# GothiProCoder/OCR-System

Measured on AMD Instinct MI355X. Metric: pages/sec end-to-end det+rec, A4@200DPI, higher is better.
Workload: dtype bf16; 1 GPU; end-to-end det+rec, batch=64 A4@200DPI pages per GPU (BASELINE configs[3]); pages_per_gpu=64, global_batch=64, lines_last_step=3279, pages_gathered_last_step=64, parallelism=pages sharded dp1, 1 all-gather/step, ranks=1, input=pages pre-decoded (uint8 RGB) and resident in HBM when the timed region starts, det_sub_batch=64

## Files before the change

### include/lumina_ocr.h

```cpp
#ifndef LUMINA_OCR_H
#define LUMINA_OCR_H
#include <stddef.h>
#include <stdint.h>

#ifdef __cplusplus
extern "C" {
#endif

typedef struct lumina_ocr lumina_ocr_t;

#define LUMINA_REC_H 32
#define LUMINA_REC_W 320
#define LUMINA_REC_T 80
#define LUMINA_MAX_WORDS 40
#define LUMINA_MAX_BOXES 1000

int lumina_ocr_create(int device, lumina_ocr_t** out);
void lumina_ocr_destroy(lumina_ocr_t* h);
const char* lumina_ocr_last_error(const lumina_ocr_t* h);
const char* lumina_ocr_version(void);
int lumina_ocr_set_option(lumina_ocr_t* h, const char* key, int value);

int lumina_ocr_load_det_weights(lumina_ocr_t* h, const void* blob, size_t nbytes);
int lumina_ocr_load_rec_weights(lumina_ocr_t* h, const void* blob, size_t nbytes);
// ... 27 lines not shown
int lumina_ocr_rec_forward(lumina_ocr_t* h, const uint8_t* crops_dev, const int32_t* widths_dev, int n_crops, int32_t* idx_dev,
                           float* prob_dev, void* stream);

int lumina_ocr_ctc_decode(lumina_ocr_t* h, const int32_t* idx_dev, const float* prob_dev, int n, int32_t* text_dev, int32_t* len_dev,
                          float* score_dev, void* stream);

int lumina_ocr_ctc_decode_words(lumina_ocr_t* h, const int32_t* idx_dev, const float* prob_dev, int n, const int32_t* quads_dev,
                                const int32_t* widths_dev, const int32_t* flip_dev , int space_id, int32_t* text_dev,
                                int32_t* len_dev, float* score_dev, int32_t* word_quads_dev, int32_t* word_span_dev, float* word_score_dev,
                                int32_t* word_count_dev, void* stream);

int lumina_ocr_resize_lanczos(lumina_ocr_t* h, const uint8_t* in_dev, int n, int height, int width, int channels, uint8_t* out_dev,
                              int out_h, int out_w, void* stream);
int lumina_ocr_enhance(lumina_ocr_t* h, const uint8_t* img_dev, int n, int height, int width, float contrast, float sharpness,
                       uint8_t* tmp_dev, uint8_t* out_dev, void* stream);

int lumina_ocr_binarize(lumina_ocr_t* h, const uint8_t* img_dev, int n, int height, int width, int adaptive, int threshold, uint8_t* out_dev,
                        void* stream);

int lumina_ocr_exif_transpose(lumina_ocr_t* h, const uint8_t* img_dev, int n, int height, int width, int orientation, uint8_t* out_dev, void* stream);
int lumina_ocr_grayscale(lumina_ocr_t* h, const uint8_t* img_dev, int n, int height, int width, uint8_t* out_dev, void* stream);
int lumina_ocr_denoise(lumina_ocr_t* h, const uint8_t* img_dev, int n, int height, int width, uint8_t* out_dev, void* stream);

int lumina_ocr_deskew(lumina_ocr_t* h, const uint8_t* pages_dev, int n, int height, int width, uint8_t* out_dev, double* rot_dev,
                      int32_t* info_dev, uint8_t* edges_dev, int32_t* segs_dev, int32_t* nsegs_dev, void* stream);
int lumina_ocr_deskew_warp(lumina_ocr_t* h, const uint8_t* pages_dev, int n, int height, int width, const double* rot_dev, uint8_t* out_dev,
                           void* stream);

int lumina_ocr_table_rules(lumina_ocr_t* h, const uint8_t* pages_dev, int n, int height, int width, int threshold, int gap, int min_len,
                           int max_thick, int max_rules, int32_t* hrules_dev, int32_t* vrules_dev, int32_t* counts_dev, uint64_t* hmask_dev,
// ... 50 lines not shown
```

### ocr-system_amd/csrc/capi.hip

```cpp
#include <cstdlib>
#include <cstring>
#include <new>

#include "../../include/lumina_ocr.h"
#include "dbpost.h"
#include "deskew.h"
#include "engine.h"
#include "marks.h"
#include "ops.h"
#include "orient.h"
#include "resize.h"
#include "runs.h"
#include "jpeg.h"
#include "jpegdec.h"
#include "pngdec.h"
#include "stem_conv.h"
#include "tables.h"

#define API_TRY try {
#define API_CATCH(h)                                                             \
    }                                                                            \
    catch (const std::exception& e) { return locr_fail(h, "exception", e.what()); } \
    catch (...) { return locr_fail(h, "exception", "unknown"); }

// ... 84 lines not shown
    else if (!strcmp(key, "fuse_head")) h->fuse_head = value != 0;
    else if (!strcmp(key, "fuse_mb")) h->fuse_mb = value != 0;
    else if (!strcmp(key, "fuse_pool")) h->fuse_pool = value != 0;
    else if (!strcmp(key, "fuse_stem")) h->fuse_stem = value != 0;
    else if (!strcmp(key, "fpn_multi")) h->fpn_multi = value != 0;
    else if (!strcmp(key, "fpn_compose")) h->fpn_compose = value != 0;
    else if (!strcmp(key, "fuse_short")) h->fuse_short = value != 0;
    else if (!strcmp(key, "conv_ring")) h->conv_ring = value != 0;
    else if (!strcmp(key, "blocked_layout")) h->blocked_layout = value != 0;
    else if (!strcmp(key, "conv_big_min")) h->conv_big_min = value >= 0 ? value : 1024;
    else if (!strcmp(key, "ring_orient")) h->ring_orient = value < 0 ? -1 : (value != 0);
    else if (!strcmp(key, "post_group")) h->post_group = value > 0 ? value : 1;
    else if (!strcmp(key, "tail_group")) h->tail_group = value > 0 ? value : 0;
    else if (!strcmp(key, "svtr_f16")) h->svtr_f16 = value < 0 ? -1 : (value != 0);
    else if (!strcmp(key, "png_sub_batch_mb")) h->pd_sub_batch_mb = value > 0 ? value : 1;
    else if (!strcmp(key, "conv2d_variant")) h->conv2d_variant = value < 0 || value > 2 ? 0 : value;
    else return locr_fail(h, "set_option: unknown key", key);
    return 0;
}

int lumina_ocr_load_det_weights(lumina_ocr_t* h, const void* blob, size_t nbytes) {
    if (!h || !blob) return 1;
    BIND(h);
    API_TRY return eng_load_det(h, blob, nbytes); API_CATCH(h)
}
int lumina_ocr_load_rec_weights(lumina_ocr_t* h, const void* blob, size_t nbytes) {
    if (!h || !blob) return 1;
    BIND(h);
    API_TRY return eng_load_rec(h, blob, nbytes); API_CATCH(h)
}
// ... 194 lines not shown
    auto it = h->coeff_cache.find(key);
    if (it == h->coeff_cache.end()) {
        std::vector<int> bounds, kk;
        lumina_ocr::Coeffs c;
        lanczos_coeffs(in_size, out_size, &c.ksize, &bounds, &kk);
        c.bounds_host = std::make_shared<std::vector<int>>(bounds);
        c.bounds = static_cast<int*>(eng_upload(h, bounds.data(), bounds.size() * 4));
        c.kk = static_cast<int*>(eng_upload(h, kk.data(), kk.size() * 4));
        if (!c.bounds || !c.kk) return locr_fail(h, "resize", "coefficient table upload");
        it = h->coeff_cache.emplace(key, c).first;
    }
    *out = it->second;
    return 0;
}

int lumina_ocr_resize_lanczos(lumina_ocr_t* h, const uint8_t* in_dev, int n, int height, int width, int channels, uint8_t* out_dev,
                              int out_h, int out_w, void* stream) {
    if (!h || !in_dev || !out_dev || n <= 0 || height <= 0 || width <= 0 || out_h <= 0 || out_w <= 0 || channels <= 0)
        return locr_fail(h, "resize_lanczos", "bad arguments");
    BIND(h);
    API_TRY
    hipStream_t st = (hipStream_t)stream;
    const uint8_t* src = in_dev;
    int cur_w = width;
    const bool need_h = out_w != width, need_v = out_h != height;
    if (!need_h && !need_v) {
        return hip_rc(h, "resize_lanczos", hipMemcpyAsync(out_dev, in_dev, (size_t)n * height * width * channels, hipMemcpyDeviceToDevice, st));
    }
    if (need_h) {
        lumina_ocr::Coeffs c;
        if (get_coeffs(h, width, out_w, &c)) return 1;
        uint8_t* dst = out_dev;
        if (need_v) {
            if (hip_rc(h, "resize_lanczos", h->aux.reserve((size_t)n * height * out_w * channels))) return 1;
            dst = h->aux.get();
        }
        if (hip_rc(h, "resize_lanczos", resample_launch(src, dst, c.bounds, c.kk, c.ksize, n, height, width, channels, out_w, 0, c.bounds_host->data(), st))) return 1;
        src = dst; cur_w = out_w;
    }
    if (need_v) {
        lumina_ocr::Coeffs c;
        if (get_coeffs(h, height, out_h, &c)) return 1;
        if (hip_rc(h, "resize_lanczos", resample_launch(src, out_dev, c.bounds, c.kk, c.ksize, n, height, cur_w, channels, out_h, 1, c.bounds_host->data(), st))) return 1;
    }
    return 0;
    API_CATCH(h)
}

int lumina_ocr_enhance(lumina_ocr_t* h, const uint8_t* img_dev, int n, int height, int width, float contrast, float sharpness,
                       uint8_t* tmp_dev, uint8_t* out_dev, void* stream) {
    if (!h || !img_dev || !tmp_dev || !out_dev || n <= 0) return locr_fail(h, "enhance", "bad arguments");
    BIND(h);
    if (hip_rc(h, "enhance", h->sums.reserve(sizeof(unsigned long long) * (size_t)n))) return 1;
    unsigned long long* sums = reinterpret_cast<unsigned long long*>(h->sums.get());
    return hip_rc(h, "enhance", enhance_launch(img_dev, tmp_dev, out_dev, sums, n, height, width, contrast, sharpness, (hipStream_t)stream));
}

int lumina_ocr_binarize(lumina_ocr_t* h, const uint8_t* img_dev, int n, int height, int width, int adaptive, int threshold, uint8_t* out_dev, void* stream) {
    if (!h || !img_dev || !out_dev || n <= 0 || height <= 0 || width <= 0) return locr_fail(h, "binarize", "bad arguments");
    BIND(h);
    return hip_rc(h, "binarize", binarize_launch(img_dev, out_dev, n, height, width, adaptive != 0, threshold, (hipStream_t)stream));
}

int lumina_ocr_exif_transpose(lumina_ocr_t* h, const uint8_t* img_dev, int n, int height, int width, int orientation, uint8_t* out_dev, void* stream) {
    if (!h || !img_dev || !out_dev || n <= 0 || height <= 0 || width <= 0 || orientation < 1 || orientation > 8 || img_dev == out_dev)
        return locr_fail(h, "exif_transpose", "bad arguments (orientation 1..8, not in place)");
    BIND(h);
    return hip_rc(h, "exif_transpose", exif_transpose_launch(img_dev, out_dev, n, height, width, orientation, (hipStream_t)stream));
}

// ... 280 lines not shown
```

### ocr-system_amd/csrc/engine.h

```cpp
#pragma once
#include <map>
#include <memory>
#include <string>
#include <type_traits>
#include <vector>

#include "common.h"
#include "conv_mfma.h"
#include "mbconv.h"
#include "svtr.h"

struct Tensor4 {
    bf16_t* p = nullptr;
    int n = 0, h = 0, w = 0, c = 0;
    bool blk = false;
    int n_src = 0; const bf16_t* xs[4] = {nullptr, nullptr, nullptr, nullptr}; int xs_shift[4] = {0, 0, 0, 0};
    int xs_c[4] = {0, 0, 0, 0}, xs_cs[4] = {0, 0, 0, 0};
    int src_c(int k) const { return xs_c[k] ? xs_c[k] : c / n_src; }
    int src_cs(int k) const { return xs_cs[k] ? xs_cs[k] : src_c(k); }
    size_t elems() const { return (size_t)n * h * w * c; }
};

struct ConvLayer {
    std::string name;
// ... 103 lines not shown
    bool blocked_layout = true;
    bool conv_ring = true;
    int svtr_f16 = -1;
    int conv2d_variant = 0;
    int ring_orient = -1;
    bool fuse_short = true;
    bool fpn_compose = true;
    bool fpn_multi = true;
    bool fuse_stem = true;
    bool fuse_mb = true;
    bool time_convs = false;
    std::vector<LaunchRecord> launches;
    struct Coeffs { int ksize = 0; int* bounds = nullptr; int* kk = nullptr; std::shared_ptr<std::vector<int>> bounds_host; };
    std::map<std::pair<int, int>, Coeffs> coeff_cache;
    Growable<DeviceMem> aux;
    Growable<DeviceMem> sums;
    int jd_last_passes = 0;
    struct Staging { Growable<PinnedMem> buf; Event uploaded; };
    Staging jd_stage[2];
    int jd_stage_next = 0;
    Staging pd_stage;
    int pd_sub_batch_mb = 768;
    float* dk_trig = nullptr; short* dk_wtab = nullptr;
};

int locr_fail(lumina_ocr* eng, const char* what, const char* detail);
bool parse_blob(lumina_ocr* eng, const void* blob, size_t n, std::map<std::string, HostBlobTensor>* out);

int eng_load_det(lumina_ocr* eng, const void* blob, size_t n);
int eng_load_rec(lumina_ocr* eng, const void* blob, size_t n);
int eng_det_forward(lumina_ocr* eng, const uint8_t* pages, int B, int H, int W, int Hp, int Wp, bf16_t* prob, hipStream_t st);
// ... 11 lines not shown
```

### ocr-system_amd/csrc/resize.h

```cpp
#pragma once
#include <vector>

#include "common.h"

void lanczos_coeffs(int in_size, int out_size, int* ksize_out, std::vector<int>* bounds, std::vector<int>* kk);
hipError_t resample_launch(const uint8_t* in, uint8_t* out, const int* bounds_dev, const int* kk_dev, int ksize, int N, int H, int W, int C,
                           int out_len, int axis, const int* bounds_host, hipStream_t st);
hipError_t enhance_launch(const uint8_t* img, uint8_t* tmp, uint8_t* out, unsigned long long* sums_dev, int N, int H, int W, float contrast,
                          float sharpness, hipStream_t st);
hipError_t binarize_launch(const uint8_t* img, uint8_t* out, int N, int H, int W, int adaptive, int threshold, hipStream_t st);
hipError_t grayscale_launch(const uint8_t* img, uint8_t* out, int N, int H, int W, hipStream_t st);
hipError_t median3_launch(const uint8_t* img, uint8_t* out, int N, int H, int W, hipStream_t st);
hipError_t exif_transpose_launch(const uint8_t* img, uint8_t* out, int N, int H, int W, int orientation, hipStream_t st);
```

### ocr-system_amd/csrc/resize.hip

```cpp
#include "resize.h"
#include "lds_rows.h"

#include <cmath>

namespace {

constexpr int PRECISION_BITS = 32 - 8 - 2;

__global__ __launch_bounds__(256) void resample_h_kernel(const uint8_t* in, uint8_t* out, const int* bounds, const int* kk, int ksize, int H, int W,
                                                         int C, int Wo, size_t total_bytes) {
    extern __shared__ uint32_t row_lds[];
    const int row = blockIdx.x;
    const size_t start = (size_t)row * W * C;
    const int off = (int)(start & 3);
    const uint32_t* src = reinterpret_cast<const uint32_t*>(in + (start - off));
    const int nwords = (off + W * C + 3) >> 2;
    const size_t wbase = start - off;
    for (int i = threadIdx.x; i < nwords; i += 256) {
        uint32_t w;
        if (wbase + 4 * (size_t)(i + 1) <= total_bytes) w = src[i];
        else {
            w = 0;
            for (int b = 0; b < 4; ++b)
                if (wbase + 4 * (size_t)i + b < total_bytes) w |= (uint32_t)in[wbase + 4 * (size_t)i + b] << (8 * b);
// ... 167 lines not shown
            const uint32_t w = __builtin_amdgcn_alignbyte(lr[1], lr[0], (uint32_t)(off & 3));
            const int kj = kl[rr * VK + j];
            s0 += __mul24((int)(w & 0xff), kj); s1 += __mul24((int)((w >> 8) & 0xff), kj); s2 += __mul24((int)((w >> 16) & 0xff), kj); s3 += __mul24((int)(w >> 24), kj);
        }
        s0 >>= PRECISION_BITS; s1 >>= PRECISION_BITS; s2 >>= PRECISION_BITS; s3 >>= PRECISION_BITS;
        const uint32_t res = (uint32_t)(s0 < 0 ? 0 : (s0 > 255 ? 255 : s0)) | ((uint32_t)(s1 < 0 ? 0 : (s1 > 255 ? 255 : s1)) << 8) |
                             ((uint32_t)(s2 < 0 ? 0 : (s2 > 255 ? 255 : s2)) << 16) | ((uint32_t)(s3 < 0 ? 0 : (s3 > 255 ? 255 : s3)) << 24);
        uint8_t* dst = out + go - mo + 4 * tid;
        if (ew >= 0 && ew + 4 <= rowbytes) *reinterpret_cast<uint32_t*>(dst) = res;
        else
            for (int j = 0; j < 4; ++j)
                if (ew + j >= 0 && ew + j < rowbytes) dst[j] = (uint8_t)(res >> (8 * j));
    }
}

__global__ __launch_bounds__(256) void gray_sum_kernel(const uint8_t* img, unsigned long long* sums, int HW) {
    __shared__ unsigned long long part[4];
    const int n = blockIdx.y;
    const uint8_t* p = img + (size_t)n * HW * 3;
    unsigned long long s = 0;
    for (int i = blockIdx.x * blockDim.x + threadIdx.x; i < HW; i += gridDim.x * blockDim.x) {
        const unsigned r = p[(size_t)i * 3], g = p[(size_t)i * 3 + 1], b = p[(size_t)i * 3 + 2];
        s += (r * 19595u + g * 38470u + b * 7471u + 0x8000u) >> 16;
    }
    for (int m = 32; m >= 1; m >>= 1) {
        const unsigned lo = __shfl_xor((unsigned)(s & 0xffffffffull), m), hi = __shfl_xor((unsigned)(s >> 32), m);
        s += ((unsigned long long)hi << 32) | lo;
    }
    if ((threadIdx.x & 63) == 0) part[threadIdx.x >> 6] = s;
    __syncthreads();
// ... 171 lines not shown
        if (bounds_host != nullptr && ksize <= VKMAX && lds_bytes <= 60 * 1024) {
            const dim3 grid((rowbytes + 3 + VT_XB - 1) / VT_XB, (out_len + VT_R - 1) / VT_R, N);
            if (vk == 9) hipLaunchKernelGGL(resample_v_tile_kernel<9>, grid, dim3(256), lds_bytes, st, in, out, bounds_dev, kk_dev, ksize, H, rowbytes, out_len, (long long)N * H * rowbytes);
            else hipLaunchKernelGGL(resample_v_tile_kernel<VKMAX>, grid, dim3(256), lds_bytes, st, in, out, bounds_dev, kk_dev, ksize, H, rowbytes, out_len, (long long)N * H * rowbytes);
            return hipGetLastError();
        }
        const bool a4 = rowbytes % 4 == 0 && (reinterpret_cast<uintptr_t>(in) % 4 == 0) && (reinterpret_cast<uintptr_t>(out) % 4 == 0);
        const bool a2 = rowbytes % 2 == 0 && (reinterpret_cast<uintptr_t>(in) % 2 == 0) && (reinterpret_cast<uintptr_t>(out) % 2 == 0);
        if (a4) hipLaunchKernelGGL(resample_v_kernel<4>, dim3(N * out_len), dim3(256), 0, st, in, out, bounds_dev, kk_dev, ksize, H, rowbytes, out_len);
        else if (a2) hipLaunchKernelGGL(resample_v_kernel<2>, dim3(N * out_len), dim3(256), 0, st, in, out, bounds_dev, kk_dev, ksize, H, rowbytes, out_len);
        else hipLaunchKernelGGL(resample_v_kernel<1>, dim3(N * out_len), dim3(256), 0, st, in, out, bounds_dev, kk_dev, ksize, H, rowbytes, out_len);
    }
    return hipGetLastError();
}

namespace {
constexpr int BZ_TH = 16, BZ_TW = 64, BZ_R = 5;
__constant__ float c_gauss11[11] = {0x1.20c256p-7f, 0x1.bcb86ap-6f, 0x1.0ab50ap-4f, 0x1.f2464cp-4f, 0x1.6a7e1ep-3f, 0x1.9ac20ap-3f,
                                    0x1.6a7e1ep-3f, 0x1.f2464cp-4f, 0x1.0ab50ap-4f, 0x1.bcb86ap-6f, 0x1.20c256p-7f};
__device__ __forceinline__ int lum_L(const uint8_t* p) { return (19595 * p[0] + 38470 * p[1] + 7471 * p[2] + 0x8000) >> 16; }

__global__ __launch_bounds__(256) void binarize_kernel(const uint8_t* img, uint8_t* out, int H, int W, int adaptive, int threshold) {
    __shared__ uint8_t sL[(BZ_TH + 2 * BZ_R) * (BZ_TW + 2 * BZ_R)];
    __shared__ float sRow[(BZ_TH + 2 * BZ_R) * BZ_TW];
    const int pg = blockIdx.z, y0 = blockIdx.y * BZ_TH, x0 = blockIdx.x * BZ_TW, tid = threadIdx.x;
    const uint8_t* src = img + (size_t)pg * H * W * 3;
    uint8_t* dst = out + (size_t)pg * H * W * 3;
    constexpr int LW = BZ_TW + 2 * BZ_R, LH = BZ_TH + 2 * BZ_R;
    if (!adaptive) {
        for (int i = tid; i < BZ_TH * BZ_TW; i += 256) {
// ... 102 lines not shown
    long long g = (npix + 255) / 256;
    hipLaunchKernelGGL(grayscale_kernel, dim3((unsigned)(g > 65536 ? 65536 : g)), dim3(256), 0, st, img, out, npix);
    return hipGetLastError();
}

hipError_t median3_launch(const uint8_t* img, uint8_t* out, int N, int H, int W, hipStream_t st) {
    hipLaunchKernelGGL(median3_kernel, dim3((W + 63) / 64, (H + 3) / 4, N), dim3(256), 0, st, img, out, H, W);
    return hipGetLastError();
}

hipError_t binarize_launch(const uint8_t* img, uint8_t* out, int N, int H, int W, int adaptive, int threshold, hipStream_t st) {
    hipLaunchKernelGGL(binarize_kernel, dim3((W + BZ_TW - 1) / BZ_TW, (H + BZ_TH - 1) / BZ_TH, N), dim3(256), 0, st, img, out, H, W, adaptive, threshold);
    return hipGetLastError();
}

hipError_t enhance_launch(const uint8_t* img, uint8_t* tmp, uint8_t* out, unsigned long long* sums_dev, int N, int H, int W, float contrast,
                          float sharpness, hipStream_t st) {
    hipError_t e = hipMemsetAsync(sums_dev, 0, sizeof(unsigned long long) * N, st);
    if (e != hipSuccess) return e;
    const int HW = H * W;
    int gx = (HW + 255) / 256;
    if (gx > 2048) gx = 2048;
    hipLaunchKernelGGL(gray_sum_kernel, dim3(gx > 64 ? 64 : gx, N), dim3(256), 0, st, img, sums_dev, HW);
    (void)tmp;
    const int rowb = W * 3;
    hipLaunchKernelGGL(enhance_kernel, dim3((rowb + 3 + EN_XB - 1) / EN_XB, (H + EN_R - 1) / EN_R, N), dim3(256), 0, st, img, out, sums_dev, H, W,
                       contrast, sharpness, (long long)N * H * rowb);
    return hipGetLastError();
}
```

### ocr-system_amd/lumina_ocr/engine.py

```python
from __future__ import annotations

import ctypes
import os
from pathlib import Path
from typing import Dict, Optional, Tuple

import numpy as np

from . import arch

_LIB_PATH = Path(__file__).resolve().parent.parent / "lib" / "liblumina_ocr.so"

REC_H, REC_W, REC_T = 32, 320, 80
MAX_WORDS = 40
MAX_BOXES = 1000


class EngineUnavailable(RuntimeError):
    pass


class EngineError(RuntimeError):
    pass

# ... 25 lines not shown
        "lumina_ocr_det_postprocess": (i32, [vp, vp, i32, i32, i32, i32, i32, f32, f32, f32, i32, i32, vp, vp, vp, vp]),
        "lumina_ocr_rec_crop": (i32, [vp, vp, i32, i32, i32, vp, vp, i32, vp, vp, vp]),
        "lumina_ocr_rec_crop_oriented": (i32, [vp, vp, i32, i32, i32, vp, vp, i32, vp, vp, vp, vp]),
        "lumina_ocr_cls_crop": (i32, [vp, vp, i32, i32, i32, vp, vp, i32, vp, vp, vp]),
        "lumina_ocr_load_cls_weights": (i32, [vp, vp, sz]),
        "lumina_ocr_cls_forward": (i32, [vp, vp, vp, i32, f32, vp, vp, vp, vp]),
        "lumina_ocr_rec_forward": (i32, [vp, vp, vp, i32, vp, vp, vp]),
        "lumina_ocr_ctc_decode": (i32, [vp, vp, vp, i32, vp, vp, vp, vp]),
        "lumina_ocr_ctc_decode_words": (i32, [vp, vp, vp, i32, vp, vp, vp, i32, vp, vp, vp, vp, vp, vp, vp, vp]),
        "lumina_ocr_conv2d": (i32, [vp, vp, i32, i32, i32, i32, vp, vp, i32, i32, i32, i32, vp, vp, vp]),
        "lumina_ocr_read_tap": (i32, [vp, c.c_char_p, vp, sz, c.POINTER(i32)]),
        "lumina_ocr_conv_timing": (i32, [vp, c.POINTER(c.c_double), c.POINTER(c.c_double), c.POINTER(i32)]),
        "lumina_ocr_conv_timing_detail": (i32, [vp, c.c_char_p, sz]),
        "lumina_ocr_resize_lanczos": (i32, [vp, vp, i32, i32, i32, i32, vp, i32, i32, vp]),
        "lumina_ocr_enhance": (i32, [vp, vp, i32, i32, i32, f32, f32, vp, vp, vp]),
        "lumina_ocr_jpeg_encode": (i32, [vp, vp, i32, i32, i32, i32, i32, vp, sz, vp, vp]),
        "lumina_ocr_jpeg_probe": (i32, [vp, sz, vp]),
        "lumina_ocr_jpeg_last_passes": (i32, [vp]),
        "lumina_ocr_jpeg_decode_async": (i32, [vp, vp, vp, i32, i32, i32, vp, vp, i32, vp]),
        "lumina_ocr_jpeg_decode": (i32, [vp, vp, vp, i32, i32, i32, vp, vp, vp]),
        "lumina_ocr_jpeg_coefficients": (i32, [vp, vp, i32, i32, i32, i32, vp, vp]),
        "lumina_ocr_png_probe": (i32, [vp, sz, vp]),
        "lumina_ocr_png_decode": (i32, [vp, vp, vp, i32, i32, i32, vp, vp, vp]),
        "lumina_ocr_load_svtr_weights": (i32, [vp, vp, sz]),
        "lumina_ocr_svtr_forward": (i32, [vp, vp, vp, i32, vp, vp, vp]),
        "lumina_ocr_svtr_num_classes": (i32, [vp]),
        "lumina_ocr_svtr_dtype": (i32, [vp]),
        "lumina_ocr_binarize": (i32, [vp, vp, i32, i32, i32, i32, i32, vp, vp]),
        "lumina_ocr_grayscale": (i32, [vp, vp, i32, i32, i32, vp, vp]),
        "lumina_ocr_exif_transpose": (i32, [vp, vp, i32, i32, i32, i32, vp, vp]),
# ... 16 lines not shown
            missing.append(name)
            continue
        fn.restype = res
        fn.argtypes = args
    lib._missing = missing
    _lib = lib
    return lib


EXPORTED_SYMBOLS = [
    "lumina_ocr_create", "lumina_ocr_destroy", "lumina_ocr_last_error", "lumina_ocr_version", "lumina_ocr_set_option",
    "lumina_ocr_load_det_weights", "lumina_ocr_load_rec_weights", "lumina_ocr_num_classes", "lumina_ocr_normalize",
    "lumina_ocr_det_forward", "lumina_ocr_det_postprocess", "lumina_ocr_rec_crop", "lumina_ocr_rec_crop_oriented", "lumina_ocr_cls_crop",
    "lumina_ocr_load_cls_weights", "lumina_ocr_cls_forward", "lumina_ocr_rec_forward",
    "lumina_ocr_ctc_decode", "lumina_ocr_ctc_decode_words", "lumina_ocr_conv2d", "lumina_ocr_read_tap", "lumina_ocr_conv_timing", "lumina_ocr_conv_timing_detail",
    "lumina_ocr_resize_lanczos", "lumina_ocr_enhance", "lumina_ocr_jpeg_encode", "lumina_ocr_jpeg_coefficients", "lumina_ocr_jpeg_probe", "lumina_ocr_jpeg_decode", "lumina_ocr_jpeg_decode_async", "lumina_ocr_jpeg_last_passes",
    "lumina_ocr_png_probe", "lumina_ocr_png_decode",
    "lumina_ocr_load_svtr_weights", "lumina_ocr_svtr_forward", "lumina_ocr_svtr_num_classes", "lumina_ocr_svtr_dtype", "lumina_ocr_binarize", "lumina_ocr_exif_transpose", "lumina_ocr_grayscale", "lumina_ocr_denoise", "lumina_ocr_deskew", "lumina_ocr_deskew_warp",
    "lumina_ocr_table_rules", "lumina_ocr_selection_marks", "lumina_ocr_rules_and_marks",
    "lumina_ocr_page_quarter_workspace_bytes", "lumina_ocr_page_quarter", "lumina_ocr_page_turn", "lumina_ocr_page_vote",
]


def _torch():
    import torch
    return torch


def _ptr(t) -> int:
    return 0 if t is None else t.data_ptr()

# ... 295 lines not shown
        buf = ctypes.create_string_buffer(1 << 20)
        self._chk(self.lib.lumina_ocr_conv_timing_detail(self._h, buf, len(buf)))
        rows = []
        for line in buf.value.decode().splitlines():
            name, kern, ms, gf, mb = line.split()
            rows.append((name, kern, float(ms), float(gf), float(mb)))
        return rows

    def resize_lanczos(self, img, out_h: int, out_w: int):
        torch = _torch()
        n, h, w, c = img.shape
        out = torch.empty((n, out_h, out_w, c), dtype=torch.uint8, device=img.device)
        self._chk(self.lib.lumina_ocr_resize_lanczos(self._h, _ptr(img), n, h, w, c, _ptr(out), out_h, out_w, self._stream()))
        return out

    def deskew(self, pages, debug: bool = False, estimate_only: bool = False):
        torch = _torch()
        n, h, w, c = pages.shape
        assert c == 3 and pages.dtype == torch.uint8 and pages.is_contiguous()
        out = None if estimate_only else torch.empty_like(pages)
        rot = torch.empty((n, 3), dtype=torch.float64, device=pages.device)
        info = torch.empty((n, 2), dtype=torch.int32, device=pages.device)
        edges = segs = nsegs = None
        if debug:
            edges = torch.empty((n, h, w), dtype=torch.uint8, device=pages.device)
            segs = torch.zeros((n, 512, 8, 4), dtype=torch.int32, device=pages.device)
            nsegs = torch.zeros((n, 512), dtype=torch.int32, device=pages.device)
        self._chk(self.lib.lumina_ocr_deskew(self._h, _ptr(pages), n, h, w, _ptr(out), _ptr(rot), _ptr(info), _ptr(edges), _ptr(segs), _ptr(nsegs),
                                             self._stream()))
        return (out, rot, info, edges, segs, nsegs) if debug else (out, rot)
# ... 141 lines not shown
```

### ocr-system_amd/lumina_ocr/pipeline.py

```python
from __future__ import annotations

import logging
from dataclasses import dataclass, field
from typing import List, Optional, Sequence, Tuple

import numpy as np

from . import arch
from .engine import MAX_BOXES, Engine
from .utils import page_orient
from .utils.image_preprocessing import get_optimal_size

logger = logging.getLogger(__name__)


@dataclass
class PageDetections:
    quads: np.ndarray
    texts: List[str]
    scores: np.ndarray
    det_scores: np.ndarray
    width: int = 0
    height: int = 0
    text_ids: Optional[np.ndarray] = None
# ... 56 lines not shown
        self.mark_params = dict(arch.MARK_PARAMS if mark_params is None else mark_params)
        self.page_orient = bool(page_orient)
        self.word_boxes = bool(word_boxes)
        self.space_id = self.charset.index(" ") if " " in self.charset else -1
        self.page_orient_params = dict(arch.PAGE_ORIENT_PARAMS if page_orient_params is None else page_orient_params)
        if self.angle_cls and not engine.cls_loaded:
            raise ValueError("angle_cls needs the orientation classifier's weights (Engine.load_cls)")
        if self.page_orient and not engine.cls_loaded:
            raise ValueError("page_orient needs the orientation classifier's weights (Engine.load_cls)")
        if self.page_orient and gather is not None:
            raise ValueError("page_orient does not run with a gather: a page's turn and its processed size stay on their rank")

    def preprocess(self, pages, enhance: bool = True, deskew: bool = False):
        b, h, w, _ = pages.shape
        nw, nh = get_optimal_size(w, h, self.max_dimension)
        x = pages if (nw, nh) == (w, h) else self.eng.resize_lanczos(pages, nh, nw)
        if deskew:
            x, self.last_skew_angles = self.eng.deskew(x)
        if self.binarize:
            return self.eng.binarize(x, adaptive=self.binarize == "adaptive")
        return self.eng.enhance(x, 1.2, 1.1) if enhance else x

    def detect(self, processed):
        b, h, w, _ = processed.shape
        prob = self.eng.det_forward(processed)
        return self.eng.det_postprocess(prob, h, w, **self.post)

    def recognize(self, processed, boxes, scores, counts) -> List[PageDetections]:
        return self.finish(self.submit_recognize(processed, boxes, scores, counts))[0]

# ... 239 lines not shown
```

Before: 1540 pages/sec.

## Fuse two-pass Lanczos resize with grayscale sum into one LDS-tiled kernel

```diff
diff --git a/include/lumina_ocr.h b/include/lumina_ocr.h
--- a/include/lumina_ocr.h
+++ b/include/lumina_ocr.h
@@ -65,6 +65,9 @@
                               int out_h, int out_w, void* stream);
 int lumina_ocr_enhance(lumina_ocr_t* h, const uint8_t* img_dev, int n, int height, int width, float contrast, float sharpness,
                        uint8_t* tmp_dev, uint8_t* out_dev, void* stream);
+int lumina_ocr_preprocess(lumina_ocr_t* h, const uint8_t* in_dev, int n, int height, int width, uint8_t* resized_dev, uint8_t* out_dev, int out_h,
+                          int out_w, float contrast, float sharpness, void* stream);
+int lumina_ocr_debug_preprocess_state(lumina_ocr_t* h, unsigned long long* sums_host, int n, int* resize_path);
 
 int lumina_ocr_binarize(lumina_ocr_t* h, const uint8_t* img_dev, int n, int height, int width, int adaptive, int threshold, uint8_t* out_dev,
                         void* stream);
diff --git a/ocr-system_amd/csrc/capi.hip b/ocr-system_amd/csrc/capi.hip
--- a/ocr-system_amd/csrc/capi.hip
+++ b/ocr-system_amd/csrc/capi.hip
@@ -122,6 +122,7 @@
     else if (!strcmp(key, "tail_group")) h->tail_group = value > 0 ? value : 0;
     else if (!strcmp(key, "svtr_f16")) h->svtr_f16 = value < 0 ? -1 : (value != 0);
     else if (!strcmp(key, "png_sub_batch_mb")) h->pd_sub_batch_mb = value > 0 ? value : 1;
+    else if (!strcmp(key, "resize_fused")) h->resize_fused = value != 0;
     else if (!strcmp(key, "conv2d_variant")) h->conv2d_variant = value < 0 || value > 2 ? 0 : value;
     else return locr_fail(h, "set_option: unknown key", key);
     return 0;
@@ -346,36 +347,54 @@
     return 0;
 }
 
+static int resize_run(lumina_ocr* h, const uint8_t* in_dev, int n, int height, int width, int channels, uint8_t* out_dev, int out_h, int out_w,
+                      unsigned long long* sums_dev, bool* sums_done, const uint8_t** result, hipStream_t st) {
+    *sums_done = false;
+    h->last_resize_path = 0;
+    const bool need_h = out_w != width, need_v = out_h != height;
+    const size_t out_bytes = (size_t)n * out_h * out_w * channels;
+    const size_t inter = need_h && need_v ? ((size_t)n * height * out_w * channels + 255) / 256 * 256 : 0;
+    lumina_ocr::Coeffs ch, cv;
+    if (need_h && get_coeffs(h, width, out_w, &ch)) return 1;
+    if (need_v && get_coeffs(h, height, out_h, &cv)) return 1;
+    ResampleHvPlan plan;
+    if (need_h && need_v && h->resize_fused) plan = resample_hv_plan(ch.ksize, ch.bounds_host->data(), cv.ksize, cv.bounds_host->data(), n, channels, out_h, out_w);
+    const size_t aux_bytes = (plan.ok ? 0 : inter) + (out_dev ? 0 : out_bytes);
+    if (aux_bytes && hip_rc(h, "resize_lanczos", h->aux.reserve(aux_bytes))) return 1;
+    if (!out_dev) out_dev = h->aux.get() + (plan.ok ? 0 : inter);
+    *result = out_dev;
+    if (!need_h && !need_v) {
+        return hip_rc(h, "resize_lanczos", hipMemcpyAsync(out_dev, in_dev, out_bytes, hipMemcpyDeviceToDevice, st));
+    }
+    if (plan.ok) {
+        if (hip_rc(h, "resize_lanczos", resample_hv_launch(plan, in_dev, out_dev, ch.bounds, ch.kk, ch.ksize, cv.bounds, cv.kk, cv.ksize, n, height, width,
+                                                           out_h, out_w, sums_dev, st))) return 1;
+        *sums_done = sums_dev != nullptr;
+        h->last_resize_path = 1;
+        return 0;
+    }
+    const uint8_t* src = in_dev;
+    int cur_w = width;
+    if (need_h) {
+        uint8_t* dst = need_v ? h->aux.get() : out_dev;
+        if (hip_rc(h, "resize_lanczos", resample_launch(src, dst, ch.bounds, ch.kk, ch.ksize, n, height, width, channels, out_w, 0, ch.bounds_host->data(), st))) return 1;
+        src = dst; cur_w = out_w;
+    }
+    if (need_v) {
+        if (hip_rc(h, "resize_lanczos", resample_launch(src, out_dev, cv.bounds, cv.kk, cv.ksize, n, height, cur_w, channels, out_h, 1, cv.bounds_host->data(), st))) return 1;
+    }
+    return 0;
+}
+
 int lumina_ocr_resize_lanczos(lumina_ocr_t* h, const uint8_t* in_dev, int n, int height, int width, int channels, uint8_t* out_dev,
                               int out_h, int out_w, void* stream) {
     if (!h || !in_dev || !out_dev || n <= 0 || height <= 0 || width <= 0 || out_h <= 0 || out_w <= 0 || channels <= 0)
         return locr_fail(h, "resize_lanczos", "bad arguments");
     BIND(h);
     API_TRY
-    hipStream_t st = (hipStream_t)stream;
-    const uint8_t* src = in_dev;
-    int cur_w = width;
-    const bool need_h = out_w != width, need_v = out_h != height;
-    if (!need_h && !need_v) {
-        return hip_rc(h, "resize_lanczos", hipMemcpyAsync(out_dev, in_dev, (size_t)n * height * width * channels, hipMemcpyDeviceToDevice, st));
-    }
-    if (need_h) {
-        lumina_ocr::Coeffs c;
-        if (get_coeffs(h, width, out_w, &c)) return 1;
-        uint8_t* dst = out_dev;
-        if (need_v) {
-            if (hip_rc(h, "resize_lanczos", h->aux.reserve((size_t)n * height * out_w * channels))) return 1;
-            dst = h->aux.get();
-        }
-        if (hip_rc(h, "resize_lanczos", resample_launch(src, dst, c.bounds, c.kk, c.ksize, n, height, width, channels, out_w, 0, c.bounds_host->data(), st))) return 1;
-        src = dst; cur_w = out_w;
-    }
-    if (need_v) {
-        lumina_ocr::Coeffs c;
-        if (get_coeffs(h, height, out_h, &c)) return 1;
-        if (hip_rc(h, "resize_lanczos", resample_launch(src, out_dev, c.bounds, c.kk, c.ksize, n, height, cur_w, channels, out_h, 1, c.bounds_host->data(), st))) return 1;
-    }
-    return 0;
+    bool sums_done;
+    const uint8_t* result;
+    return resize_run(h, in_dev, n, height, width, channels, out_dev, out_h, out_w, nullptr, &sums_done, &result, (hipStream_t)stream);
     API_CATCH(h)
 }
 
@@ -385,7 +404,36 @@
     BIND(h);
     if (hip_rc(h, "enhance", h->sums.reserve(sizeof(unsigned long long) * (size_t)n))) return 1;
     unsigned long long* sums = reinterpret_cast<unsigned long long*>(h->sums.get());
-    return hip_rc(h, "enhance", enhance_launch(img_dev, tmp_dev, out_dev, sums, n, height, width, contrast, sharpness, (hipStream_t)stream));
+    return hip_rc(h, "enhance", enhance_launch(img_dev, tmp_dev, out_dev, sums, false, n, height, width, contrast, sharpness, (hipStream_t)stream));
+}
+
+int lumina_ocr_preprocess(lumina_ocr_t* h, const uint8_t* in_dev, int n, int height, int width, uint8_t* resized_dev, uint8_t* out_dev, int out_h,
+                          int out_w, float contrast, float sharpness, void* stream) {
+    if (!h || !in_dev || !out_dev || n <= 0 || height <= 0 || width <= 0 || out_h <= 0 || out_w <= 0 || resized_dev == out_dev)
+        return locr_fail(h, "preprocess", "bad arguments");
+    BIND(h);
+    API_TRY
+    hipStream_t st = (hipStream_t)stream;
+    if (hip_rc(h, "preprocess", h->sums.reserve(sizeof(unsigned long long) * (size_t)n))) return 1;
+    unsigned long long* sums = reinterpret_cast<unsigned long long*>(h->sums.get());
+    const uint8_t* resized = in_dev;
+    bool sums_done = false;
+    if (out_h != height || out_w != width) {
+        if (hip_rc(h, "preprocess", hipMemsetAsync(sums, 0, sizeof(unsigned long long) * (size_t)n, st))) return 1;
+        if (resize_run(h, in_dev, n, height, width, 3, resized_dev, out_h, out_w, sums, &sums_done, &resized, st)) return 1;
+    }
+    return hip_rc(h, "preprocess", enhance_launch(resized, nullptr, out_dev, sums, sums_done, n, out_h, out_w, contrast, sharpness, st));
+    API_CATCH(h)
+}
+
+int lumina_ocr_debug_preprocess_state(lumina_ocr_t* h, unsigned long long* sums_host, int n, int* resize_path) {
+    if (!h || (sums_host && n <= 0)) return locr_fail(h, "debug_preprocess_state", "bad arguments");
+    BIND(h);
+    if (resize_path) *resize_path = h->last_resize_path;
+    if (!sums_host) return 0;
+    if (!h->sums.get() || h->sums.cap < sizeof(unsigned long long) * (size_t)n) return locr_fail(h, "debug_preprocess_state", "no enhance / preprocess call of that many pages yet");
+    if (hipDeviceSynchronize() != hipSuccess) return locr_fail(h, "debug_preprocess_state", "sync failed");
+    return hip_rc(h, "debug_preprocess_state", hipMemcpy(sums_host, h->sums.get(), sizeof(unsigned long long) * (size_t)n, hipMemcpyDeviceToHost));
 }
 
 int lumina_ocr_binarize(lumina_ocr_t* h, const uint8_t* img_dev, int n, int height, int width, int adaptive, int threshold, uint8_t* out_dev, void* stream) {
diff --git a/ocr-system_amd/csrc/engine.h b/ocr-system_amd/csrc/engine.h
--- a/ocr-system_amd/csrc/engine.h
+++ b/ocr-system_amd/csrc/engine.h
@@ -141,7 +141,9 @@
     struct Coeffs { int ksize = 0; int* bounds = nullptr; int* kk = nullptr; std::shared_ptr<std::vector<int>> bounds_host; };
     std::map<std::pair<int, int>, Coeffs> coeff_cache;
     Growable<DeviceMem> aux;
+    bool resize_fused = true;
     Growable<DeviceMem> sums;
+    int last_resize_path = -1;
     int jd_last_passes = 0;
     struct Staging { Growable<PinnedMem> buf; Event uploaded; };
     Staging jd_stage[2];
diff --git a/ocr-system_amd/csrc/resize.h b/ocr-system_amd/csrc/resize.h
--- a/ocr-system_amd/csrc/resize.h
+++ b/ocr-system_amd/csrc/resize.h
@@ -6,8 +6,13 @@
 void lanczos_coeffs(int in_size, int out_size, int* ksize_out, std::vector<int>* bounds, std::vector<int>* kk);
 hipError_t resample_launch(const uint8_t* in, uint8_t* out, const int* bounds_dev, const int* kk_dev, int ksize, int N, int H, int W, int C,
                            int out_len, int axis, const int* bounds_host, hipStream_t st);
-hipError_t enhance_launch(const uint8_t* img, uint8_t* tmp, uint8_t* out, unsigned long long* sums_dev, int N, int H, int W, float contrast,
-                          float sharpness, hipStream_t st);
+struct ResampleHvPlan { bool ok = false; int p_in = 0, nr_max = 0; size_t lds_bytes = 0; };
+ResampleHvPlan resample_hv_plan(int ksize_h, const int* bounds_h_host, int ksize_v, const int* bounds_v_host, int N, int C, int Ho, int Wo);
+hipError_t resample_hv_launch(const ResampleHvPlan& p, const uint8_t* in, uint8_t* out, const int* bounds_h_dev, const int* kk_h_dev, int ksize_h,
+                              const int* bounds_v_dev, const int* kk_v_dev, int ksize_v, int N, int H, int W, int Ho, int Wo,
+                              unsigned long long* sums_dev, hipStream_t st);
+hipError_t enhance_launch(const uint8_t* img, uint8_t* tmp, uint8_t* out, unsigned long long* sums_dev, bool sums_given, int N, int H, int W,
+                          float contrast, float sharpness, hipStream_t st);
 hipError_t binarize_launch(const uint8_t* img, uint8_t* out, int N, int H, int W, int adaptive, int threshold, hipStream_t st);
 hipError_t grayscale_launch(const uint8_t* img, uint8_t* out, int N, int H, int W, hipStream_t st);
 hipError_t median3_launch(const uint8_t* img, uint8_t* out, int N, int H, int W, hipStream_t st);
diff --git a/ocr-system_amd/csrc/resize.hip b/ocr-system_amd/csrc/resize.hip
--- a/ocr-system_amd/csrc/resize.hip
+++ b/ocr-system_amd/csrc/resize.hip
@@ -205,6 +205,113 @@
     }
 }
 
+constexpr int FT_X = 84, FT_Y = 40, FP_MID = 67;
+template <int FK>
+__global__ __launch_bounds__(256) void resample_hv_rgb_kernel(const uint8_t* in, uint8_t* out, const int* __restrict__ bounds_h,
+                                                              const int* __restrict__ kk_h, int ksize_h, const int* __restrict__ bounds_v,
+                                                              const int* __restrict__ kk_v, int ksize_v, int H, int W, int Ho, int Wo, int p_in,
+                                                              int nr_max, long long total_in, unsigned long long* sums) {
+    constexpr int FW = (3 * FK + 3 + 3) / 4;
+    extern __shared__ uint32_t lds[];
+    __shared__ unsigned part[4];
+    uint32_t* lin = lds;
+    uint32_t* mid = lds + nr_max * p_in;
+    const int tid = threadIdx.x;
+    const int n = blockIdx.z, yo0 = blockIdx.y * FT_Y, xo0 = blockIdx.x * FT_X;
+    const int nx = min(FT_X, Wo - xo0), ny = min(FT_Y, Ho - yo0);
+    const int rgrp = tid / FT_X, xi = tid - rgrp * FT_X;
+    const int xo = xo0 + min(xi, nx - 1);
+    const int lo = bounds_h[2 * xo];
+    int kreg[FK];
+#pragma unroll
+    for (int j = 0; j < FK; ++j) kreg[j] = j < ksize_h ? kk_h[(size_t)xo * ksize_h + j] : 0;
+    const int px_lo = bounds_h[2 * xo0];
+    const int px_hi = bounds_h[2 * (xo0 + nx - 1)] + bounds_h[2 * (xo0 + nx - 1) + 1];
+    const int r_lo = bounds_v[2 * yo0];
+    const int nr = bounds_v[2 * (yo0 + ny - 1)] + bounds_v[2 * (yo0 + ny - 1) + 1] - r_lo;
+    const int rowb = W * 3;
+    const long long g0 = (((long long)n * H + r_lo) * W + px_lo) * 3;
+    const int nw = ((px_hi - px_lo) * 3 + 3 + 3) / 4;
+    fill_rows(lin, p_in, nw, in, g0, rowb, nr, 0, nr, total_in, WordIdentity());
+    __syncthreads();
+    const uintptr_t ibase = reinterpret_cast<uintptr_t>(in), obase = reinterpret_cast<uintptr_t>(out);
+    const int m0 = (int)((ibase + (unsigned long long)g0) & 3), dm = rowb & 3;
+    if (rgrp < 3 && xi < nx) {
+        uint8_t* mb = reinterpret_cast<uint8_t*>(mid) + 4 + xi * 3;
+        const int pb = (lo - px_lo) * 3;
+#pragma unroll 2
+        for (int r = rgrp; r < nr; r += 3) {
+            const int off = ((m0 + r * dm) & 3) + pb;
+            const uint32_t* lr = lin + r * p_in + (off >> 2);
+            const uint32_t sh = (uint32_t)(off & 3);
+            uint32_t w[FW];
+#pragma unroll
+            for (int i = 0; i < FW; ++i) w[i] = lr[i];
+            uint32_t a[FW - 1];
+#pragma unroll
+            for (int i = 0; i < FW - 1; ++i) a[i] = __builtin_amdgcn_alignbyte(w[i + 1], w[i], sh);
+            int s0 = 1 << (PRECISION_BITS - 1), s1 = s0, s2 = s0;
+#pragma unroll
+            for (int j = 0; j < FK; ++j) {
+                s0 += __mul24((int)((a[(3 * j) >> 2] >> (8 * ((3 * j) & 3))) & 0xffu), kreg[j]);
+                s1 += __mul24((int)((a[(3 * j + 1) >> 2] >> (8 * ((3 * j + 1) & 3))) & 0xffu), kreg[j]);
+                s2 += __mul24((int)((a[(3 * j + 2) >> 2] >> (8 * ((3 * j + 2) & 3))) & 0xffu), kreg[j]);
+            }
+            s0 >>= PRECISION_BITS; s1 >>= PRECISION_BITS; s2 >>= PRECISION_BITS;
+            uint8_t* o = mb + r * (FP_MID * 4);
+            o[0] = (uint8_t)(s0 < 0 ? 0 : (s0 > 255 ? 255 : s0));
+            o[1] = (uint8_t)(s1 < 0 ? 0 : (s1 > 255 ? 255 : s1));
+            o[2] = (uint8_t)(s2 < 0 ? 0 : (s2 > 255 ? 255 : s2));
+        }
+    }
+    __syncthreads();
+    const int wv = __builtin_amdgcn_readfirstlane(tid >> 6), lane = tid & 63;
+    const int segb = nx * 3;
+    unsigned gs = 0;
+    for (int rr = wv; rr < ny; rr += 4) {
+        const int yo = yo0 + rr;
+        const int vlo = bounds_v[2 * yo] - r_lo;
+        const int* kv = kk_v + (size_t)yo * ksize_v;
+        const long long go = (((long long)n * Ho + yo) * Wo + xo0) * 3;
+        const int mo = (int)((obase + (unsigned long long)go) & 3);
+        const int b0 = 4 * lane - mo;
+        const int off = 4 + b0;
+        const uint32_t* lr = mid + vlo * FP_MID + (off >> 2);
+        const uint32_t sh = (uint32_t)(off & 3);
+        int s0 = 1 << (PRECISION_BITS - 1), s1 = s0, s2 = s0, s3 = s0;
+#pragma unroll
+        for (int j = 0; j < FK; ++j) {
+            const uint32_t w = __builtin_amdgcn_alignbyte(lr[j * FP_MID + 1], lr[j * FP_MID], sh);
+            const int kj = j < ksize_v ? kv[j] : 0;
+            s0 += __mul24((int)(w & 0xff), kj); s1 += __mul24((int)((w >> 8) & 0xff), kj); s2 += __mul24((int)((w >> 16) & 0xff), kj); s3 += __mul24((int)(w >> 24), kj);
+        }
+        s0 >>= PRECISION_BITS; s1 >>= PRECISION_BITS; s2 >>= PRECISION_BITS; s3 >>= PRECISION_BITS;
+        const uint32_t res = (uint32_t)(s0 < 0 ? 0 : (s0 > 255 ? 255 : s0)) | ((uint32_t)(s1 < 0 ? 0 : (s1 > 255 ? 255 : s1)) << 8) |
+                             ((uint32_t)(s2 < 0 ? 0 : (s2 > 255 ? 255 : s2)) << 16) | ((uint32_t)(s3 < 0 ? 0 : (s3 > 255 ? 255 : s3)) << 24);
+        uint8_t* dst = out + go + b0;
+        if (b0 >= 0 && b0 + 4 <= segb) *reinterpret_cast<uint32_t*>(dst) = res;
+        else
+            for (int j = 0; j < 4; ++j)
+                if (b0 + j >= 0 && b0 + j < segb) dst[j] = (uint8_t)(res >> (8 * j));
+        if (sums != nullptr) {
+            const uint32_t nxt = (uint32_t)__shfl_down((int)res, 1);
+            const int d = (3 - (b0 + 3) % 3) % 3;
+            const uint32_t p1 = __builtin_amdgcn_alignbyte(nxt, res, (uint32_t)d);
+            const uint32_t p2 = __builtin_amdgcn_alignbyte(nxt, res, 3u);
+            const unsigned l1 = ((p1 & 0xff) * 19595u + ((p1 >> 8) & 0xff) * 38470u + ((p1 >> 16) & 0xff) * 7471u + 0x8000u) >> 16;
+            const unsigned l2 = ((p2 & 0xff) * 19595u + ((p2 >> 8) & 0xff) * 38470u + ((p2 >> 16) & 0xff) * 7471u + 0x8000u) >> 16;
+            if (b0 + d >= 0 && b0 + d < segb) gs += l1;
+            if (d == 0 && b0 + 3 < segb) gs += l2;
+        }
+    }
+    if (sums != nullptr) {
+        for (int m = 32; m >= 1; m >>= 1) gs += __shfl_xor(gs, m);
+        if (lane == 0) part[wv] = gs;
+        __syncthreads();
+        if (tid == 0) atomicAdd(&sums[n], (unsigned long long)part[0] + part[1] + part[2] + part[3]);
+    }
+}
+
 __global__ __launch_bounds__(256) void gray_sum_kernel(const uint8_t* img, unsigned long long* sums, int HW) {
     __shared__ unsigned long long part[4];
     const int n = blockIdx.y;
@@ -406,6 +513,38 @@
     return hipGetLastError();
 }
 
+ResampleHvPlan resample_hv_plan(int ksize_h, const int* bounds_h_host, int ksize_v, const int* bounds_v_host, int N, int C, int Ho, int Wo) {
+    constexpr int FK = 9, FW = (3 * FK + 3 + 3) / 4;
+    ResampleHvPlan p;
+    if (C != 3 || ksize_h > FK || ksize_v > FK || bounds_h_host == nullptr || bounds_v_host == nullptr || N > 65535) return p;
+    int npx_max = 0, nr_max = 0;
+    for (int x0 = 0; x0 < Wo; x0 += FT_X) {
+        const int x1 = (x0 + FT_X < Wo ? x0 + FT_X : Wo) - 1;
+        const int sp = bounds_h_host[2 * x1] + bounds_h_host[2 * x1 + 1] - bounds_h_host[2 * x0];
+        if (sp > npx_max) npx_max = sp;
+    }
+    for (int y0 = 0; y0 < Ho; y0 += FT_Y) {
+        const int y1 = (y0 + FT_Y < Ho ? y0 + FT_Y : Ho) - 1;
+        const int sp = bounds_v_host[2 * y1] + bounds_v_host[2 * y1 + 1] - bounds_v_host[2 * y0];
+        if (sp > nr_max) nr_max = sp;
+    }
+    p.p_in = ((3 + 3 * npx_max) / 4 + FW + 1) | 1;
+    p.nr_max = nr_max;
+    p.lds_bytes = ((size_t)nr_max * p.p_in + (size_t)(nr_max + FK) * FP_MID) * 4;
+    p.ok = p.lds_bytes <= 48 * 1024;
+    return p;
+}
+
+hipError_t resample_hv_launch(const ResampleHvPlan& p, const uint8_t* in, uint8_t* out, const int* bounds_h_dev, const int* kk_h_dev, int ksize_h,
+                              const int* bounds_v_dev, const int* kk_v_dev, int ksize_v, int N, int H, int W, int Ho, int Wo,
+                              unsigned long long* sums_dev, hipStream_t st) {
+    if (!p.ok) return hipErrorInvalidValue;
+    const dim3 grid((Wo + FT_X - 1) / FT_X, (Ho + FT_Y - 1) / FT_Y, N);
+    hipLaunchKernelGGL(resample_hv_rgb_kernel<9>, grid, dim3(256), p.lds_bytes, st, in, out, bounds_h_dev, kk_h_dev, ksize_h, bounds_v_dev, kk_v_dev,
+                       ksize_v, H, W, Ho, Wo, p.p_in, p.nr_max, (long long)N * H * W * 3, sums_dev);
+    return hipGetLastError();
+}
+
 namespace {
 constexpr int BZ_TH = 16, BZ_TW = 64, BZ_R = 5;
 __constant__ float c_gauss11[11] = {0x1.20c256p-7f, 0x1.bcb86ap-6f, 0x1.0ab50ap-4f, 0x1.f2464cp-4f, 0x1.6a7e1ep-3f, 0x1.9ac20ap-3f,
@@ -538,14 +677,16 @@
     return hipGetLastError();
 }
 
-hipError_t enhance_launch(const uint8_t* img, uint8_t* tmp, uint8_t* out, unsigned long long* sums_dev, int N, int H, int W, float contrast,
-                          float sharpness, hipStream_t st) {
-    hipError_t e = hipMemsetAsync(sums_dev, 0, sizeof(unsigned long long) * N, st);
-    if (e != hipSuccess) return e;
-    const int HW = H * W;
-    int gx = (HW + 255) / 256;
-    if (gx > 2048) gx = 2048;
-    hipLaunchKernelGGL(gray_sum_kernel, dim3(gx > 64 ? 64 : gx, N), dim3(256), 0, st, img, sums_dev, HW);
+hipError_t enhance_launch(const uint8_t* img, uint8_t* tmp, uint8_t* out, unsigned long long* sums_dev, bool sums_given, int N, int H, int W,
+                          float contrast, float sharpness, hipStream_t st) {
+    if (!sums_given) {
+        hipError_t e = hipMemsetAsync(sums_dev, 0, sizeof(unsigned long long) * N, st);
+        if (e != hipSuccess) return e;
+        const int HW = H * W;
+        int gx = (HW + 255) / 256;
+        if (gx > 2048) gx = 2048;
+        hipLaunchKernelGGL(gray_sum_kernel, dim3(gx > 64 ? 64 : gx, N), dim3(256), 0, st, img, sums_dev, HW);
+    }
     (void)tmp;
     const int rowb = W * 3;
     hipLaunchKernelGGL(enhance_kernel, dim3((rowb + 3 + EN_XB - 1) / EN_XB, (H + EN_R - 1) / EN_R, N), dim3(256), 0, st, img, out, sums_dev, H, W,
diff --git a/ocr-system_amd/lumina_ocr/engine.py b/ocr-system_amd/lumina_ocr/engine.py
--- a/ocr-system_amd/lumina_ocr/engine.py
+++ b/ocr-system_amd/lumina_ocr/engine.py
@@ -63,6 +63,8 @@
         "lumina_ocr_conv_timing_detail": (i32, [vp, c.c_char_p, sz]),
         "lumina_ocr_resize_lanczos": (i32, [vp, vp, i32, i32, i32, i32, vp, i32, i32, vp]),
         "lumina_ocr_enhance": (i32, [vp, vp, i32, i32, i32, f32, f32, vp, vp, vp]),
+        "lumina_ocr_preprocess": (i32, [vp, vp, i32, i32, i32, vp, vp, i32, i32, f32, f32, vp]),
+        "lumina_ocr_debug_preprocess_state": (i32, [vp, vp, i32, vp]),
         "lumina_ocr_jpeg_encode": (i32, [vp, vp, i32, i32, i32, i32, i32, vp, sz, vp, vp]),
         "lumina_ocr_jpeg_probe": (i32, [vp, sz, vp]),
         "lumina_ocr_jpeg_last_passes": (i32, [vp]),
@@ -109,7 +111,7 @@
     "lumina_ocr_det_forward", "lumina_ocr_det_postprocess", "lumina_ocr_rec_crop", "lumina_ocr_rec_crop_oriented", "lumina_ocr_cls_crop",
     "lumina_ocr_load_cls_weights", "lumina_ocr_cls_forward", "lumina_ocr_rec_forward",
     "lumina_ocr_ctc_decode", "lumina_ocr_ctc_decode_words", "lumina_ocr_conv2d", "lumina_ocr_read_tap", "lumina_ocr_conv_timing", "lumina_ocr_conv_timing_detail",
-    "lumina_ocr_resize_lanczos", "lumina_ocr_enhance", "lumina_ocr_jpeg_encode", "lumina_ocr_jpeg_coefficients", "lumina_ocr_jpeg_probe", "lumina_ocr_jpeg_decode", "lumina_ocr_jpeg_decode_async", "lumina_ocr_jpeg_last_passes",
+    "lumina_ocr_resize_lanczos", "lumina_ocr_enhance", "lumina_ocr_preprocess", "lumina_ocr_debug_preprocess_state", "lumina_ocr_jpeg_encode", "lumina_ocr_jpeg_coefficients", "lumina_ocr_jpeg_probe", "lumina_ocr_jpeg_decode", "lumina_ocr_jpeg_decode_async", "lumina_ocr_jpeg_last_passes",
     "lumina_ocr_png_probe", "lumina_ocr_png_decode",
     "lumina_ocr_load_svtr_weights", "lumina_ocr_svtr_forward", "lumina_ocr_svtr_num_classes", "lumina_ocr_svtr_dtype", "lumina_ocr_binarize", "lumina_ocr_exif_transpose", "lumina_ocr_grayscale", "lumina_ocr_denoise", "lumina_ocr_deskew", "lumina_ocr_deskew_warp",
     "lumina_ocr_table_rules", "lumina_ocr_selection_marks", "lumina_ocr_rules_and_marks",
@@ -435,6 +437,29 @@
         self._chk(self.lib.lumina_ocr_resize_lanczos(self._h, _ptr(img), n, h, w, c, _ptr(out), out_h, out_w, self._stream()))
         return out
 
+    def preprocess(self, img, out_h: int, out_w: int, contrast: float = 1.2, sharpness: float = 1.1, return_resized: bool = False):
+        torch = _torch()
+        n, h, w, c = img.shape
+        assert c == 3 and img.dtype == torch.uint8
+        out = torch.empty((n, out_h, out_w, 3), dtype=torch.uint8, device=img.device)
+        resized = torch.empty_like(out) if return_resized else None
+        self._chk(self.lib.lumina_ocr_preprocess(self._h, _ptr(img), n, h, w, _ptr(resized), _ptr(out), out_h, out_w,
+                                                 contrast, sharpness, self._stream()))
+        return (out, resized) if return_resized else out
+
+    def gray_sums(self, n: int):
+        import numpy as np
+        out = np.zeros(n, np.uint64)
+        self._chk(self.lib.lumina_ocr_debug_preprocess_state(self._h, out.ctypes.data, n, None))
+        return out
+
+    def last_resize_fused(self) -> bool:
+        import ctypes
+        path = ctypes.c_int(-1)
+        self._chk(self.lib.lumina_ocr_debug_preprocess_state(self._h, None, 0, ctypes.addressof(path)))
+        assert path.value >= 0, "no resize yet"
+        return path.value == 1
+
     def deskew(self, pages, debug: bool = False, estimate_only: bool = False):
         torch = _torch()
         n, h, w, c = pages.shape
diff --git a/ocr-system_amd/lumina_ocr/pipeline.py b/ocr-system_amd/lumina_ocr/pipeline.py
--- a/ocr-system_amd/lumina_ocr/pipeline.py
+++ b/ocr-system_amd/lumina_ocr/pipeline.py
@@ -94,6 +94,8 @@
     def preprocess(self, pages, enhance: bool = True, deskew: bool = False):
         b, h, w, _ = pages.shape
         nw, nh = get_optimal_size(w, h, self.max_dimension)
+        if (nw, nh) != (w, h) and enhance and not deskew and not self.binarize:
+            return self.eng.preprocess(pages, nh, nw, 1.2, 1.1)
         x = pages if (nw, nh) == (w, h) else self.eng.resize_lanczos(pages, nh, nw)
         if deskew:
             x, self.last_skew_angles = self.eng.deskew(x)
```

Measured after the change: 1566 pages/sec, median of 6. +1.7%, better.
